# wenxiaoshuai/Points-Matching

Hardware: AMD Instinct MI355X
Metric: descriptor-pair distances/s (BF-L2 2-NN + ratio stage); RANSAC hypotheses/s in `ransac` (higher is better)
Workload: dtype f32

## Files before the change

### include/pm.h

```cpp
#ifndef PM_H_
#define PM_H_

#include <stddef.h>
#include <stdint.h>

#ifdef __cplusplus
extern "C" {
#endif

#define PM_VERSION_MAJOR 0
#define PM_VERSION_MINOR 1

typedef enum pm_status {
    PM_OK            =  0,
    PM_E_INVALID     = -1,
    PM_E_TOO_FEW     = -2,
    PM_E_NO_MODEL    = -3,
    PM_E_HIP         = -4,
    PM_E_NOMEM       = -5,
    PM_E_UNSUPPORTED = -6
} pm_status;

typedef struct pm_match {
    int32_t queryIdx;
    int32_t trainIdx;
    int32_t imgIdx;
    float   distance;
} pm_match;

typedef struct pm_ctx pm_ctx;

int  pm_ctx_create(int device, pm_ctx** out);
int  pm_ctx_destroy(pm_ctx* ctx);
int  pm_ctx_set_stream(pm_ctx* ctx, void* hip_stream);
int  pm_ctx_synchronize(pm_ctx* ctx);
int  pm_device_alloc(pm_ctx* ctx, size_t bytes, void** d_out);
int  pm_device_free(pm_ctx* ctx, void* d_ptr);
int  pm_device_upload(pm_ctx* ctx, void* d_dst, const void* src, size_t bytes);
int  pm_device_download(pm_ctx* ctx, void* dst, const void* d_src, size_t bytes);
int  pm_ctx_timing_enable(pm_ctx* ctx, int enable);
int  pm_ctx_timing_reset(pm_ctx* ctx);
int  pm_ctx_timing_get(pm_ctx* ctx, const char* kernel, double* mean_ms, int* launches);
int  pm_ctx_knn_diag_enable(pm_ctx* ctx, int enable);
int  pm_ctx_knn_stats(pm_ctx* ctx, int* rescans, int* nonfinite);
int  pm_ctx_knn_route(pm_ctx* ctx, int* route);
int  pm_ctx_filter_fusion_status(pm_ctx* ctx, int* gave_up);
enum {
    PM_OPT_RANSAC_PATH    = 1,
    PM_OPT_SCORE_OPERANDS = 2,
    PM_OPT_HAMMING_ROUTE  = 3,
    PM_OPT_KNN_F16_WAVES  = 4,
    PM_OPT_KNN_STAGING    = 6,
    PM_OPT_KNN_WG_PER_CU  = 7,
    PM_OPT_FILTER_FUSION  = 5,
    PM_OPT_KNN_XCD_TILE   = 8,
    PM_OPT_KNN_GENERAL_F16 = 9,
    PM_OPT_KNN_SEEDED     = 10,
    PM_OPT_KNN_U8_GROUP   = 11,
    PM_OPT_KNN_RING       = 12,
    PM_OPT_KNN_U8_REFINE  = 13,
    PM_OPT_KNN_RING_PROLOGUE = 14,
    PM_OPT_KNN_WIDE       = 15,
    PM_OPT_KNN_PREP_ROWS  = 16,
    PM_OPT_RANSAC_FORM    = 17,
    PM_OPT_RANSAC_WG_IDS  = 18,
    PM_OPT_HAMMING_REFINE = 19,
    PM_OPT_KNN_SUPERTILE  = 20,
    PM_OPT_FEAT_CAPACITY  = 21,
    PM_OPT_COUNT_         = 22
};
int  pm_ctx_set_option(pm_ctx* ctx, int option, int value);
int  pm_ctx_get_option(pm_ctx* ctx, int option, int* value);
const char* pm_last_error(void);
const char* pm_status_string(int status);
int  pm_version(void);

#define PM_MAX_K 16
#define PM_KNN_FORCE_EXACT  1
#define PM_KNN_FORCE_F32    2
#define PM_KNN_HINT_INTEGER 4
#define PM_KNN_HINT_U8      8
#define PM_KNN_HINT_UNIT_NORM 16
int pm_bf_knn_l2_f32(pm_ctx* ctx, const float* q, int nq, const float* t, int nt,
                     int dim, int k, int flags, pm_match* out);
int pm_bf_knn_l2_f32_dev(pm_ctx* ctx, const float* d_q, int nq, const float* d_t, int nt,
                         int dim, int k, int flags, pm_match* d_out);

int pm_bf_knn_l2_u8(pm_ctx* ctx, const uint8_t* q, int nq, const uint8_t* t, int nt, int dim, int k, pm_match* out);
int pm_bf_knn_l2_u8_dev(pm_ctx* ctx, const uint8_t* d_q, int nq, const uint8_t* d_t, int nt, int dim, int k, pm_match* d_out);
int pm_bf_knn_l2_u8_ratio_dev(pm_ctx* ctx, const uint8_t* d_q, int nq, const uint8_t* d_t, int nt, int dim, float ratio,
                              const float* d_kp1_xy, const float* d_kp2_xy, pm_match* d_knn, pm_match* d_good,
                              float* d_xy1, float* d_xy2, int32_t* d_n_good);

int pm_bf_knn_l2_ratio_dev(pm_ctx* ctx, const float* d_q, int nq, const float* d_t, int nt, int dim, int flags,
                           float ratio, const float* d_kp1_xy, const float* d_kp2_xy, pm_match* d_knn,
                           pm_match* d_good, float* d_xy1, float* d_xy2, int32_t* d_n_good);

typedef struct pm_flann_params {
    int32_t  trees;
    int32_t  checks;
    uint64_t seed;
} pm_flann_params;
typedef struct pm_flann_index pm_flann_index;
int pm_flann_build(pm_ctx* ctx, const float* train, int nt, int dim, const pm_flann_params* prm, pm_flann_index** out);
int pm_flann_destroy(pm_flann_index* ix);
int pm_flann_knn_l2_f32(pm_ctx* ctx, pm_flann_index* ix, const float* q, int nq, int k, pm_match* out);
int pm_flann_knn_l2_f32_dev(pm_ctx* ctx, pm_flann_index* ix, const float* d_q, int nq, int k, pm_match* d_out);
int pm_flann_export(const pm_flann_index* ix, int32_t* n_nodes, int32_t* roots, void* nodes, int32_t cap_nodes);

int pm_bf_knn_hamming_u8(pm_ctx* ctx, const uint8_t* q, int nq, const uint8_t* t, int nt,
                         int bytes, int k, pm_match* out);
int pm_bf_knn_hamming_u8_dev(pm_ctx* ctx, const uint8_t* d_q, int nq, const uint8_t* d_t, int nt,
                             int bytes, int k, pm_match* d_out);

int pm_pad_rows_u8(const uint8_t* src, int n, int bytes, uint8_t* dst, int dst_bytes);
int pm_pad_rows_u8_dev(pm_ctx* ctx, const uint8_t* d_src, int n, int bytes, uint8_t* d_dst, int dst_bytes);


int pm_filter_midpoint(const pm_match* m, int n, double* min_out, double* max_out,
                       pm_match* out, int* n_out);
int pm_filter_ratio(const pm_match* knn, int nq, int k, float ratio, pm_match* out, int* n_out);
int pm_filter_ratio_gather_dev(pm_ctx* ctx, const pm_match* d_knn, int nq, int k, float ratio,
// ... 311 lines not shown
```

### points_matching_amd/api.py

```python
import ctypes as C
import os

import numpy as np

_HERE = os.path.dirname(os.path.abspath(__file__))
LIB_PATH = os.environ.get("PM_LIB_PATH") or os.path.join(_HERE, "libpm_hip.so")

MATCH_DTYPE = np.dtype([("queryIdx", "<i4"), ("trainIdx", "<i4"), ("imgIdx", "<i4"),
                        ("distance", "<f4")])
PM_MAX_K = 16
PM_KNN_FORCE_EXACT = 1
PM_KNN_FORCE_F32 = 2
PM_KNN_HINT_INTEGER = 4
PM_KNN_HINT_U8 = 8
PM_KNN_HINT_UNIT_NORM = 16
PM_CROSS_RATIO_FWD = 1
PM_CROSS_RATIO_REV = 2
PM_GUIDE_F_SAMPSON = 0
PM_GUIDE_F_SYM = 1
PM_GUIDE_H = 2
PM_ERR_SAMPSON = 0
PM_ERR_SYM_EPIPOLAR = 1
PM_ERR_REPROJ = 2
PM_AFFINE_FULL = 0
# ... 54 lines not shown
    _fields_ = [("hyp_begin", C.c_int64), ("hyp_end", C.c_int64), ("seed", C.c_uint64),
                ("thresh_px", C.c_float), ("error_kind", C.c_int32)]


class PointsView(C.Structure):
    _fields_ = [("xy1", C.c_void_p), ("xy2", C.c_void_p), ("counts", C.c_void_p), ("parts", C.c_int32),
                ("cap", C.c_int32), ("pitch_xy", C.c_int64), ("pitch_cnt", C.c_int32), ("reserved", C.c_int32)]


class Camera(C.Structure):
    _fields_ = [("fx", C.c_double), ("fy", C.c_double), ("cx", C.c_double), ("cy", C.c_double)]


def _camera(K):
    if isinstance(K, Camera):
        return K
    k = np.asarray(K, np.float64)
    if k.shape == (3, 3):
        return Camera(k[0, 0], k[1, 1], k[0, 2], k[1, 2])
    return Camera(*[float(v) for v in k.reshape(4)])


class PnpView(C.Structure):
    _fields_ = [("xyz", C.c_void_p), ("uv", C.c_void_p), ("count", C.c_void_p), ("cap", C.c_int32), ("reserved", C.c_int32)]


class HRefineInfo(C.Structure):
    _fields_ = [("cost_in", C.c_double), ("cost_out", C.c_double), ("n_used", C.c_int32), ("iters", C.c_int32),
                ("status", C.c_int32), ("reserved", C.c_int32)]


H_REFINE_INFO_DTYPE = np.dtype([("cost_in", "<f8"), ("cost_out", "<f8"), ("n_used", "<i4"), ("iters", "<i4"),
                                ("status", "<i4"), ("reserved", "<i4")])

RANSAC_RECORD_DTYPE = np.dtype([("key", "<u8"), ("F", "<f8", (9,))])
PM_MAX_PARTS = 64
PM_OPT_RANSAC_PATH, PM_OPT_SCORE_OPERANDS, PM_OPT_HAMMING_ROUTE, PM_OPT_KNN_F16_WAVES, PM_OPT_FILTER_FUSION = 1, 2, 3, 4, 5
PM_OPT_KNN_STAGING = 6
PM_OPT_KNN_WG_PER_CU = 7
PM_OPT_KNN_XCD_TILE = 8
PM_OPT_KNN_GENERAL_F16 = 9
PM_OPT_KNN_SEEDED = 10
PM_OPT_KNN_U8_GROUP = 11
PM_OPT_KNN_RING = 12
PM_OPT_KNN_U8_REFINE = 13
PM_OPT_KNN_RING_PROLOGUE = 14
PM_OPT_KNN_WIDE = 15
PM_OPT_KNN_PREP_ROWS = 16
PM_OPT_RANSAC_FORM = 17
PM_OPT_RANSAC_WG_IDS = 18
PM_OPT_HAMMING_REFINE = 19
PM_OPT_KNN_SUPERTILE = 20
PM_OPT_FEAT_CAPACITY = 21


_lib = None


def lib():
    global _lib
    if _lib is None:
        if not os.path.exists(LIB_PATH):
            raise PmError(PM_E_UNSUPPORTED,
                          "%s is missing: run `python -m points_matching_amd.build`" % LIB_PATH)
        try:
            import torch
        except ImportError:
            pass
        _lib = C.CDLL(LIB_PATH)
        _lib.pm_last_error.restype = C.c_char_p
        _lib.pm_status_string.restype = C.c_char_p
        _lib.pm_format_match_list.restype = C.c_long
    return _lib


def _check(rc):
    if rc != PM_OK:
        raise PmError(rc, (lib().pm_last_error() or b"").decode() or
                      lib().pm_status_string(rc).decode())


def _p(a):
    return a.ctypes.data_as(C.c_void_p) if a is not None else None


def _pair(xy1, xy2):
    xy1 = np.ascontiguousarray(xy1, np.float32).reshape(-1, 2)
    xy2 = np.ascontiguousarray(xy2, np.float32).reshape(-1, 2)
    if xy2.shape[0] != xy1.shape[0]:
        raise ValueError("xy1 and xy2 must have the same length")
    return xy1, xy2, xy1.shape[0]


def _outcome(rc):
    if rc not in (PM_OK, PM_E_NO_MODEL, PM_E_TOO_FEW):
        _check(rc)
    return rc


def ransac_key(inliers, hyp):
    return (int(inliers) << 32) | (0xFFFFFFFF - int(hyp))


def ransac_key_hyp(key):
    return 0xFFFFFFFF - (int(key) & 0xFFFFFFFF)

# ... 1016 lines not shown
```

### points_matching_amd/csrc/ransac_fused_kernels.hpp

```cpp
#pragma once
#include <type_traits>

#include "ransac_core.hpp"
#include "ransac_internal.hpp"

namespace pm_ransac {
namespace {

constexpr int RF_THREADS = 256;
constexpr int RF_TEAMS = 2;
constexpr int RF_WG = RF_THREADS * RF_TEAMS;
constexpr int RF_PTS_PER_SLOT = 2 * RF_THREADS;
constexpr int RF_PPT2 = 5;
constexpr int RF_PPT2_BIG = 10;
static_assert(RF_PPT2_BIG <= 10, "score_tile is instantiated for 1..10 slots");

struct RfSlot {
    unsigned long long key;
    double F[9];
    unsigned long long pad[6];
};
static_assert(sizeof(RfSlot) == 128, "slot stride");

struct RfOut {
    int shard;
    unsigned long long* key;
    double* F;
    uint8_t* mask;
    int mask_len;
    int* n_inliers;
    FinalOut* fo;
    union {
        pm_ransac_record* rec;
        const double* cand;
    };
};

__device__ __forceinline__ int view_count1(const pm_points_view& v)
{
    int c = v.cap;
    if (v.counts) { const int raw = *v.counts; c = raw < 0 ? 0 : (raw > v.cap ? v.cap : raw); }
    return c;
}
__device__ __forceinline__ void view_offsets(const pm_points_view& v, int* __restrict__ offs, int tid)
{
    if (tid < 64) {
        int c = 0;
        if (tid < v.parts) {
            c = v.cap;
            if (v.counts) {
                const int raw = v.counts[static_cast<size_t>(tid) * v.pitch_cnt];
                c = raw < 0 ? 0 : (raw > v.cap ? v.cap : raw);
            }
        }
        int incl = c;
#pragma unroll
        for (int o = 1; o < 64; o <<= 1) {
            const int up = __shfl_up(incl, o, 64);
            if (tid >= o) incl += up;
        }
        if (tid < v.parts) offs[tid] = incl - c;
        if (tid == v.parts - 1) offs[v.parts] = incl;
    }
}

__device__ __forceinline__ void view_point(const pm_points_view& v, const int* __restrict__ offs, int i, float2& a, float2& b)
{
    size_t e = 2 * static_cast<size_t>(i);
    if (v.parts > 1) {
        int p = 0;
        while (p + 1 < v.parts && i >= offs[p + 1]) ++p;
        e = static_cast<size_t>(p) * static_cast<size_t>(v.pitch_xy) + 2 * static_cast<size_t>(i - offs[p]);
    }
    a = *reinterpret_cast<const float2*>(v.xy1 + e);
    b = *reinterpret_cast<const float2*>(v.xy2 + e);
}

template <typename DIAG>
__device__ __forceinline__ bool hyp_model_view(const pm_points_view& v, const int* __restrict__ offs, int n, uint64_t seed,
                                               uint64_t h, double (&F)[9])
{
    int idx[8];
    DIAG::solve(5);
    sample8(seed, h, n, idx);
    DIAG::solve(6);
    double x1[8], y1[8], x2[8], y2[8];
#pragma unroll
    for (int i = 0; i < 8; ++i) {
        float2 a, b;
// ... 95 lines not shown
                                           const f32x2 (&YP)[PPT2], float thr2, bool first, int lane, int wave, int team)
{
    if (team >= hcount) return;
    f32x4v m0 = *reinterpret_cast<const f32x4v*>(&mdl[team][0]);
    f32x4v m1 = *reinterpret_cast<const f32x4v*>(&mdl[team][4]);
    f32x2 m2 = *reinterpret_cast<const f32x2*>(&mdl[team][8]);
    for (int s = team; s < hcount; s += RF_TEAMS) {
        const f32x4v c0 = m0, c1 = m1;
        const f32x2 c2 = m2;
        const int sn = s + RF_TEAMS < hcount ? s + RF_TEAMS : s;
        m0 = *reinterpret_cast<const f32x4v*>(&mdl[sn][0]);
        m1 = *reinterpret_cast<const f32x4v*>(&mdl[sn][4]);
        m2 = *reinterpret_cast<const f32x2*>(&mdl[sn][8]);
        const ModelS ms = model_to_sgprs(c0, c1, c2);
        unsigned long long va[KM], vb[KM];
        const float fs[9] = {c0[0], c0[1], c0[2], c0[3], c1[0], c1[1], c1[2], c1[3], c2[0]};
#pragma unroll
        for (int k = 0; k < KM; ++k) {
            bool ia, ib;
            if constexpr (DIAG::scalar_fma) {
                ia = inlier32<KIND>(fs, X[k][0], Y[k][0], XP[k][0], YP[k][0], thr2);
                ib = inlier32<KIND>(fs, X[k][1], Y[k][1], XP[k][1], YP[k][1], thr2);
            } else {
                inlier_pk_model<KIND>(ms, X[k], Y[k], XP[k], YP[k], thr2, ia, ib);
            }
            va[k] = __ballot(ia);
            vb[k] = __ballot(ib);
        }
        int c = 0;
#pragma unroll
        for (int k = 0; k < KM; ++k) c += __popcll(va[k]) + __popcll(vb[k]);
        if (lane == 0) {
            if (first) cnt[wave][s] = c;
            else __hip_atomic_fetch_add(&cnt[wave][s], c, __ATOMIC_RELAXED, __HIP_MEMORY_SCOPE_WORKGROUP);
        }
    }
}

template <int NWAVES>
__device__ __forceinline__ unsigned long long wg_max_u64(unsigned long long key, unsigned long long* __restrict__ wk, int tid)
{
    key = pm::wave_max_u64(key);
    __syncthreads();
    if ((tid & 63) == 0) wk[tid >> 6] = key;
    __syncthreads();
    unsigned long long k = wk[0];
#pragma unroll
    for (int w = 1; w < NWAVES; ++w) k = wk[w] > k ? wk[w] : k;
    return k;
}

template <int KIND, int PPT2, typename DIAG>
__global__ __launch_bounds__(RF_WG) void ransac_fused(pm_points_view v, uint64_t seed, int64_t hyp_begin, int nh, int hb,
                                                           float thr2, RfSlot* __restrict__ slots, int* __restrict__ ticket,
                                                           RfOut out)
{
    __shared__ __attribute__((aligned(16))) float s_mdl[RF_HB_MAX][12];
    __shared__ double s_m64[RF_HB_MAX][9];
    __shared__ int s_cnt[RF_THREADS / 64][RF_HB_MAX];
    __shared__ int s_offs[PM_MAX_PARTS + 1];
    __shared__ unsigned long long s_wk[RF_WG / 64];
    __shared__ double s_F64[9];
    __shared__ int s_role;
    __shared__ int s_wc[RF_THREADS / 64];

    const int tid = threadIdx.x, lane = tid & 63, wave = tid >> 6;
    const int team = tid / RF_THREADS, ttid = tid % RF_THREADS, twave = wave % (RF_THREADS / 64);
    DIAG::phase(0);
    int n;
    if (v.parts == 1) {
        n = view_count1(v);
    } else {
        view_offsets(v, s_offs, tid);
        __syncthreads();
        n = s_offs[v.parts];
    }
    DIAG::phase(1);

    constexpr int RF_TILE = RF_PTS_PER_SLOT * PPT2;
    const int ntiles = n > RF_TILE ? (n + RF_TILE - 1) / RF_TILE : 1;
    f32x2 X[PPT2], Y[PPT2], XP[PPT2], YP[PPT2];
    const float nanv = __builtin_nanf("");
    auto load_tile = [&](int t) -> int {
        const int base = t * RF_TILE;
        int kmax = (n - base + RF_PTS_PER_SLOT - 1) / RF_PTS_PER_SLOT;
        kmax = kmax < 0 ? 0 : (kmax > PPT2 ? PPT2 : kmax);
#pragma unroll
        for (int k = 0; k < PPT2; ++k) {
            X[k] = f32x2{nanv, nanv}; Y[k] = X[k]; XP[k] = X[k]; YP[k] = X[k];
            if (k < kmax) {
                const int i0 = base + 2 * (k * RF_THREADS + ttid);
                float2 a0 = {nanv, nanv}, b0 = a0, a1 = a0, b1 = a0;
                if (v.parts == 1) {
                    const int j0 = i0 < n ? i0 : n - 1, j1 = i0 + 1 < n ? i0 + 1 : n - 1;
                    a0 = *reinterpret_cast<const float2*>(v.xy1 + 2 * static_cast<size_t>(j0));
                    a1 = *reinterpret_cast<const float2*>(v.xy1 + 2 * static_cast<size_t>(j1));
                    b0 = *reinterpret_cast<const float2*>(v.xy2 + 2 * static_cast<size_t>(j0));
                    b1 = *reinterpret_cast<const float2*>(v.xy2 + 2 * static_cast<size_t>(j1));
                    if (i0 >= n) { a0 = float2{nanv, nanv}; b0 = a0; }
                    if (i0 + 1 >= n) { a1 = float2{nanv, nanv}; b1 = a1; }
                } else {
                    if (i0 < n) view_point(v, s_offs, i0, a0, b0);
                    if (i0 + 1 < n) view_point(v, s_offs, i0 + 1, a1, b1);
                }
                X[k] = f32x2{a0.x, a1.x}; Y[k] = f32x2{a0.y, a1.y};
                XP[k] = f32x2{b0.x, b1.x}; YP[k] = f32x2{b0.y, b1.y};
            }
        }
        return kmax;
    };
    DIAG::phase(2);

    const int h0 = static_cast<int>(blockIdx.x) * hb;
    const int hcount = nh - h0 < hb ? nh - h0 : hb;
    if (tid < hcount) {
        double F[9];
        bool ok = false;
#pragma unroll
        for (int i = 0; i < 9; ++i) F[i] = 0.0;
        if (n >= 8) ok = hyp_model_view<DIAG>(v, s_offs, n, seed, static_cast<uint64_t>(hyp_begin + h0 + tid), F);
#pragma unroll
        for (int i = 0; i < 9; ++i) { s_mdl[tid][i] = static_cast<float>(F[i]); s_m64[tid][i] = F[i]; }
        s_mdl[tid][9] = ok ? 1.f : 0.f;
        s_mdl[tid][10] = 0.f; s_mdl[tid][11] = 0.f;
    }
    DIAG::phase(3);
    int kmax = load_tile(0);
    __syncthreads();
    DIAG::phase(4);

    for (int t = 0; t < ntiles; ++t) {
        if (t > 0) kmax = load_tile(t);
        switch (kmax) {
#define PM_CASE(KM_) case KM_: score_tile<KIND, PPT2, (KM_ <= PPT2 ? KM_ : PPT2), DIAG>(s_mdl, s_cnt, hcount, X, Y, XP, YP, thr2, t == 0, lane, twave, team); break;
            PM_CASE(1) PM_CASE(2) PM_CASE(3) PM_CASE(4) PM_CASE(5) PM_CASE(6) PM_CASE(7) PM_CASE(8) PM_CASE(9) PM_CASE(10)
#undef PM_CASE
            default:
                if (team == 0) for (int s = lane; s < hcount; s += 64) s_cnt[twave][s] = t == 0 ? 0 : s_cnt[twave][s];
                break;
        }
    }
    DIAG::phase(5);
    __syncthreads();

    unsigned long long key = 0ull;
    if (tid < hcount && s_mdl[tid][9] != 0.f) {
        int c = 0;
#pragma unroll
        for (int w = 0; w < RF_THREADS / 64; ++w) c += s_cnt[w][tid];
        key = (static_cast<unsigned long long>(static_cast<uint32_t>(c)) << 32) |
              static_cast<unsigned long long>(0xFFFFFFFFu - static_cast<uint32_t>(hyp_begin + h0 + tid));
    }
    const unsigned long long kbest = wg_max_u64<RF_WG / 64>(key, s_wk, tid);
    if (wave == 0) {
        const int sb = kbest ? static_cast<int>(static_cast<int64_t>(0xFFFFFFFFu - static_cast<uint32_t>(kbest)) - hyp_begin) - h0 : 0;
        RfSlot* sl = slots + blockIdx.x;
        if (lane < 9) __hip_atomic_store(&sl->F[lane], kbest ? s_m64[sb][lane] : 0.0, __ATOMIC_RELAXED, __HIP_MEMORY_SCOPE_AGENT);
        if (lane == 9) __hip_atomic_store(&sl->key, kbest, __ATOMIC_RELAXED, __HIP_MEMORY_SCOPE_AGENT);
        asm volatile("s_waitcnt vmcnt(0)" ::: "memory");
        if (lane == 0) {
            const int tk = __hip_atomic_fetch_add(ticket, 1, __ATOMIC_RELAXED, __HIP_MEMORY_SCOPE_AGENT);
            s_role = tk == static_cast<int>(gridDim.x) - 1 ? 1 : 0;
        }
    }
    __syncthreads();
    DIAG::phase(6);
    if (s_role == 0) { DIAG::phase(9); return; }

    if (tid == 0) __hip_atomic_store(ticket, 0, __ATOMIC_RELAXED, __HIP_MEMORY_SCOPE_AGENT);
    unsigned long long kb = 0ull;
    double fb[9];
#pragma unroll
    for (int i = 0; i < 9; ++i) fb[i] = 0.0;
    for (int j = tid; j < static_cast<int>(gridDim.x); j += RF_WG) {
        const unsigned long long kj = __hip_atomic_load(&slots[j].key, __ATOMIC_RELAXED, __HIP_MEMORY_SCOPE_AGENT);
        double fj[9];
#pragma unroll
        for (int i = 0; i < 9; ++i) fj[i] = __hip_atomic_load(&slots[j].F[i], __ATOMIC_RELAXED, __HIP_MEMORY_SCOPE_AGENT);
        if (kj > kb) {
            kb = kj;
#pragma unroll
            for (int i = 0; i < 9; ++i) fb[i] = fj[i];
        }
    }
    const unsigned long long kwin = wg_max_u64<RF_WG / 64>(kb, s_wk, tid);
    const bool ok = kwin != 0ull && n >= 8;
    if (tid < 9) s_F64[tid] = 0.0;
    __syncthreads();
    if (ok && kb == kwin) {
#pragma unroll
        for (int i = 0; i < 9; ++i) s_F64[i] = fb[i];
    }
    __syncthreads();
    DIAG::phase(7);
    if (out.shard) {
        if (tid < 9) out.rec->F[tid] = s_F64[tid];
        if (tid == 9) out.rec->key = ok ? kwin : 0ull;
        return;
    }
    if (tid < 9) {
        if (out.F) out.F[tid] = s_F64[tid];
        if (out.fo) { out.fo->F[tid] = s_F64[tid]; out.fo->F32[tid] = static_cast<float>(s_F64[tid]); }
    }
    if (tid == 9) {
        *out.key = ok ? kwin : 0ull;
        if (out.fo) out.fo->valid = ok ? 1 : 0;
    }
    float fw[9];
#pragma unroll
    for (int i = 0; i < 9; ++i) fw[i] = static_cast<float>(s_F64[i]);
    int mine = 0;
    if (team == 0) {
        for (int t = 0; t < ntiles; ++t) {
            if (ntiles > 1) kmax = load_tile(t);
#pragma unroll
            for (int k = 0; k < PPT2; ++k) {
                if (k < kmax) {
                    bool ia, ib;
                    inlier32_x2_flags<KIND>(fw, X[k], Y[k], XP[k], YP[k], thr2, ia, ib);
                    ia = ia && ok; ib = ib && ok;
                    const int i0 = t * RF_TILE + 2 * (k * RF_THREADS + ttid);
                    if (i0 < out.mask_len) out.mask[i0] = ia ? 1 : 0;
                    if (i0 + 1 < out.mask_len) out.mask[i0 + 1] = ib ? 1 : 0;
                    mine += __popcll(__ballot(ia)) + __popcll(__ballot(ib));
                }
            }
        }
        if (lane == 0) s_wc[twave] = mine;
    }
    const int covered = n > 0 ? (n + RF_PTS_PER_SLOT - 1) / RF_PTS_PER_SLOT * RF_PTS_PER_SLOT : 0;
    for (int i = covered + tid; i < out.mask_len; i += RF_WG) out.mask[i] = 0;
    __syncthreads();
    if (tid == 0) {
        int tot = 0;
#pragma unroll
        for (int w = 0; w < RF_THREADS / 64; ++w) tot += s_wc[w];
        if (out.n_inliers) *out.n_inliers = tot;
        if (out.fo) out.fo->n_inliers = tot;
    }
    DIAG::phase(8);
    DIAG::phase(9);
}

constexpr int RL_WAVES = 12;
constexpr int RL_THREADS = RL_WAVES * 64;
constexpr int RL_SLOT_PTS = 128;
constexpr int RL_MAX_SLOTS = 64;

struct GeomF {
    static constexpr bool OWN = false;
    static constexpr int PLANES = 4, MW = 12, FLAG = 9, WORDS = 9, MAX_SLOTS = RL_MAX_SLOTS;
};
template <typename M, typename = void>
struct GeomOf {
    using type = GeomF;
};
template <typename M>
struct GeomOf<M, std::void_t<typename M::Geom>> {
    using type = typename M::Geom;
};

template <typename MODEL, int NH>
__device__ __forceinline__ void score_lds(const float (*s_mdl)[12], int* s_cnt, const f32x2* pp, int kslots, int s0, float thr2, int lane)
{
    ModelS ms[NH];
    int c[NH];
#pragma unroll
    for (int h = 0; h < NH; ++h) {
        const float* m = s_mdl[s0 + h * RL_WAVES];
        ms[h] = model_to_sgprs(*reinterpret_cast<const f32x4v*>(m), *reinterpret_cast<const f32x4v*>(m + 4),
                               *reinterpret_cast<const f32x2*>(m + 8));
        c[h] = 0;
    }
    for (int slot = 0; slot < kslots; ++slot) {
        const f32x2 x = pp[0], y = pp[64], xp = pp[128], yp = pp[192];
        pp += 256;
#pragma unroll
        for (int h = 0; h < NH; ++h) {
            bool ia, ib;
            MODEL::inlier_pk(ms[h], x, y, xp, yp, thr2, ia, ib);
            c[h] += __popcll(__ballot(ia)) + __popcll(__ballot(ib));
        }
    }
    if (lane == 0) {
// ... 10 lines not shown
        typename MODEL::Regs ms[NH];
        int c[NH];
#pragma unroll
        for (int h = 0; h < NH; ++h) {
            ms[h] = MODEL::regs(s_mdl[ss[h]]);
            c[h] = 0;
        }
        for (int slot = 0; slot < kslots; ++slot) {
            f32x2 op[G::PLANES];
#pragma unroll
            for (int q = 0; q < G::PLANES; ++q) op[q] = pp[64 * q];
            pp += 64 * G::PLANES;
#pragma unroll
            for (int h = 0; h < NH; ++h) {
                bool ia, ib;
                MODEL::inlier_pk(ms[h], op, thr2, ia, ib);
                c[h] += __popcll(__ballot(ia)) + __popcll(__ballot(ib));
            }
        }
        if (lane == 0) {
#pragma unroll
            for (int h = 0; h < NH; ++h) s_cnt[ss[h]] += c[h];
        }
    } else {
        ModelS ms[NH];
        int c[NH];
#pragma unroll
        for (int h = 0; h < NH; ++h) {
            const float* m = s_mdl[ss[h]];
            ms[h] = model_to_sgprs(*reinterpret_cast<const f32x4v*>(m), *reinterpret_cast<const f32x4v*>(m + 4),
                                   *reinterpret_cast<const f32x2*>(m + 8));
            c[h] = 0;
        }
        for (int slot = 0; slot < kslots; ++slot) {
            const f32x2 x = pp[0], y = pp[64], xp = pp[128], yp = pp[192];
            pp += 256;
#pragma unroll
            for (int h = 0; h < NH; ++h) {
                bool ia, ib;
                MODEL::inlier_pk(ms[h], x, y, xp, yp, thr2, ia, ib);
                c[h] += __popcll(__ballot(ia)) + __popcll(__ballot(ib));
            }
        }
        if (lane == 0) {
#pragma unroll
            for (int h = 0; h < NH; ++h) s_cnt[ss[h]] += c[h];
        }
    }
}

template <typename MODEL, typename DIAG>
__global__ __launch_bounds__(RL_THREADS) void ransac_fused_lds(pm_points_view v, uint64_t seed, int64_t hyp_begin, int nh, int hb,
                                                               float thr2, int tile_slots, RfSlot* __restrict__ slots,
                                                               int* __restrict__ ticket, RfOut out)
{
    using G = typename GeomOf<MODEL>::type;
    extern __shared__ __attribute__((aligned(16))) f32x2 s_pts[];
    __shared__ __attribute__((aligned(16))) float s_mdl[RF_HB_MAX][G::MW];
    __shared__ double s_m64[RF_HB_MAX][G::WORDS];
    __shared__ int s_cnt[RF_HB_MAX];
    __shared__ int s_offs[PM_MAX_PARTS + 1];
    __shared__ unsigned long long s_wk[RL_WAVES];
    __shared__ double s_F64[G::WORDS];
    __shared__ int s_role;
    __shared__ int s_wc[RL_WAVES];

    const int tid = threadIdx.x, lane = tid & 63, wave = tid >> 6;
    DIAG::phase(0);
    int n;
    if (v.parts == 1) {
        n = view_count1(v);
    } else {
        view_offsets(v, s_offs, tid);
        __syncthreads();
        n = s_offs[v.parts];
    }
    DIAG::phase(1);
    const int tile_pts = tile_slots * RL_SLOT_PTS;
    const int ntiles = n > tile_pts ? (n + tile_pts - 1) / tile_pts : 1;
    const float nanv = __builtin_nanf("");
    auto load_pair = [&](int base, int slot, int l) {
        const int i0 = base + 2 * (64 * slot + l);
        if constexpr (G::OWN) {
            MODEL::load_pair(v, n, i0, s_pts + static_cast<size_t>(slot) * G::PLANES * 64 + l);
        } else {
            float2 a0 = {nanv, nanv}, b0 = a0, a1 = a0, b1 = a0;
            if (v.parts == 1) {
                if (n > 0) {
                    const int j0 = i0 < n ? i0 : n - 1, j1 = i0 + 1 < n ? i0 + 1 : n - 1;
                    a0 = *reinterpret_cast<const float2*>(v.xy1 + 2 * static_cast<size_t>(j0));
                    a1 = *reinterpret_cast<const float2*>(v.xy1 + 2 * static_cast<size_t>(j1));
                    b0 = *reinterpret_cast<const float2*>(v.xy2 + 2 * static_cast<size_t>(j0));
                    b1 = *reinterpret_cast<const float2*>(v.xy2 + 2 * static_cast<size_t>(j1));
                }
                if (i0 >= n) { a0 = float2{nanv, nanv}; b0 = a0; }
                if (i0 + 1 >= n) { a1 = float2{nanv, nanv}; b1 = a1; }
            } else {
                if (i0 < n) view_point(v, s_offs, i0, a0, b0);
                if (i0 + 1 < n) view_point(v, s_offs, i0 + 1, a1, b1);
            }
            f32x2* d = s_pts + (static_cast<size_t>(slot) * 4) * 64 + l;
            d[0] = f32x2{a0.x, a1.x}; d[64] = f32x2{a0.y, a1.y}; d[128] = f32x2{b0.x, b1.x}; d[192] = f32x2{b0.y, b1.y};
        }
    };
    auto tile_kslots = [&](int t) {
        int k = (n - t * tile_pts + RL_SLOT_PTS - 1) / RL_SLOT_PTS;
        return k < 0 ? 0 : (k > tile_slots ? tile_slots : k);
// ... 43 lines not shown

    for (int t = 0; t < ntiles; ++t) {
        const int kslots = tile_kslots(t);
        if (t > 0) {
            __syncthreads();
            for (int slot = wave; slot < kslots; slot += RL_WAVES) load_pair(t * tile_pts, slot, lane);
            __syncthreads();
        }
        if constexpr (MODEL::CANDIDATES) {
            const int sk = wave + RL_WAVES * lane;
            unsigned long long live = __ballot(sk < hcount && s_mdl[sk < hcount ? sk : 0][G::FLAG] != 0.f);
            while (live) {
                int ss[4];
                int k = 0;
#pragma unroll
                for (int h = 0; h < 4; ++h) {
                    ss[h] = wave;
                    if (live) {
                        ss[h] = wave + RL_WAVES * static_cast<int>(__builtin_ctzll(live));
                        live &= live - 1;
                        k = h + 1;
                    }
                }
                if (k == 4) score_lds_ids<MODEL, 4, G>(s_mdl, s_cnt, s_pts + lane, kslots, ss, thr2, lane);
                else if (k == 3) score_lds_ids<MODEL, 3, G>(s_mdl, s_cnt, s_pts + lane, kslots, ss, thr2, lane);
                else if (k == 2) score_lds_ids<MODEL, 2, G>(s_mdl, s_cnt, s_pts + lane, kslots, ss, thr2, lane);
                else score_lds_ids<MODEL, 1, G>(s_mdl, s_cnt, s_pts + lane, kslots, ss, thr2, lane);
            }
        } else {
            for (int s = wave; s < hcount; s += 4 * RL_WAVES) {
                const int left = (hcount - s + RL_WAVES - 1) / RL_WAVES;
                if (left >= 4) score_lds<MODEL, 4>(s_mdl, s_cnt, s_pts + lane, kslots, s, thr2, lane);
                else if (left == 3) score_lds<MODEL, 3>(s_mdl, s_cnt, s_pts + lane, kslots, s, thr2, lane);
                else if (left == 2) score_lds<MODEL, 2>(s_mdl, s_cnt, s_pts + lane, kslots, s, thr2, lane);
                else score_lds<MODEL, 1>(s_mdl, s_cnt, s_pts + lane, kslots, s, thr2, lane);
            }
        }
    }
    DIAG::phase(5);
    __syncthreads();

    unsigned long long key = 0ull;
    if (tid < hcount && s_mdl[tid][G::FLAG] != 0.f)
        key = (static_cast<unsigned long long>(static_cast<uint32_t>(s_cnt[tid])) << 32) |
              static_cast<unsigned long long>(0xFFFFFFFFu - static_cast<uint32_t>(hyp_begin + h0 + tid));
    const unsigned long long kbest = wg_max_u64<RL_WAVES>(key, s_wk, tid);
    if (wave == 0) {
        const int sb = kbest ? static_cast<int>(static_cast<int64_t>(0xFFFFFFFFu - static_cast<uint32_t>(kbest)) - hyp_begin) - h0 : 0;
        double* sf = reinterpret_cast<double*>(slots) + static_cast<size_t>(lane) * gridDim.x + blockIdx.x;
        if (lane < G::WORDS) __hip_atomic_store(sf, kbest ? s_m64[sb][lane] : 0.0, __ATOMIC_RELAXED, __HIP_MEMORY_SCOPE_AGENT);
        if (lane == G::WORDS) __hip_atomic_store(reinterpret_cast<unsigned long long*>(sf), kbest, __ATOMIC_RELAXED, __HIP_MEMORY_SCOPE_AGENT);
        asm volatile("s_waitcnt vmcnt(0)" ::: "memory");
        if (lane == 0) {
            const int tk = __hip_atomic_fetch_add(ticket, 1, __ATOMIC_RELAXED, __HIP_MEMORY_SCOPE_AGENT);
            s_role = tk == static_cast<int>(gridDim.x) - 1 ? 1 : 0;
        }
    }
    __syncthreads();
    DIAG::phase(6);
    if (s_role == 0) { DIAG::phase(9); return; }

    if (tid == 0) __hip_atomic_store(ticket, 0, __ATOMIC_RELAXED, __HIP_MEMORY_SCOPE_AGENT);
    unsigned long long kb = 0ull;
    double fb[G::WORDS];
#pragma unroll
    for (int i = 0; i < G::WORDS; ++i) fb[i] = 0.0;
    for (int j = tid; j < static_cast<int>(gridDim.x); j += RL_THREADS) {
        const double* sf = reinterpret_cast<const double*>(slots) + j;
        const unsigned long long kj = __hip_atomic_load(reinterpret_cast<const unsigned long long*>(sf + G::WORDS * static_cast<size_t>(gridDim.x)),
                                                        __ATOMIC_RELAXED, __HIP_MEMORY_SCOPE_AGENT);
        double fj[G::WORDS];
#pragma unroll
        for (int i = 0; i < G::WORDS; ++i) fj[i] = __hip_atomic_load(sf + i * static_cast<size_t>(gridDim.x), __ATOMIC_RELAXED, __HIP_MEMORY_SCOPE_AGENT);
        if (kj > kb) {
            kb = kj;
#pragma unroll
            for (int i = 0; i < G::WORDS; ++i) fb[i] = fj[i];
        }
    }
    const unsigned long long kwin = wg_max_u64<RL_WAVES>(kb, s_wk, tid);
    const bool ok = kwin != 0ull && n >= MODEL::MIN_PTS;
    if (tid < G::WORDS) s_F64[tid] = 0.0;
    __syncthreads();
    if (ok && kb == kwin) {
#pragma unroll
        for (int i = 0; i < G::WORDS; ++i) s_F64[i] = fb[i];
    }
    __syncthreads();
    DIAG::phase(7);
    if (MODEL::SHARD_OUT && out.shard) {
        if (tid < 9) out.rec->F[tid] = s_F64[tid];
        if (tid == 9) out.rec->key = ok ? kwin : 0ull;
        return;
    }
    if (tid < G::WORDS) {
        if (out.F && (MODEL::OUT_WORDS == G::WORDS || tid < MODEL::OUT_WORDS)) out.F[tid] = s_F64[tid];
        if (MODEL::SHARD_OUT && out.fo) { out.fo->F[tid] = s_F64[tid]; out.fo->F32[tid] = static_cast<float>(s_F64[tid]); }
    }
    if (tid == G::WORDS) {
        *out.key = ok ? kwin : 0ull;
        if (MODEL::SHARD_OUT && out.fo) out.fo->valid = ok ? 1 : 0;
    }
    float fw[G::OWN ? G::MW : 9];
    if constexpr (G::OWN) {
        MODEL::mask_model(out.cand, ok, kwin, hyp_begin, fw);
    } else {
#pragma unroll
        for (int i = 0; i < 9; ++i) fw[i] = static_cast<float>(s_F64[i]);
    }
    int mine = 0;
    for (int t = 0; t < ntiles; ++t) {
        const int kslots = tile_kslots(t);
        if (ntiles > 1) {
            __syncthreads();
            for (int slot = wave; slot < kslots; slot += RL_WAVES) load_pair(t * tile_pts, slot, lane);
            __syncthreads();
        }
        for (int slot = wave; slot < kslots; slot += RL_WAVES) {
            const f32x2* pp = s_pts + static_cast<size_t>(slot) * (64 * G::PLANES) + lane;
            bool ia, ib;
            if constexpr (G::OWN) {
                f32x2 op[G::PLANES];
#pragma unroll
                for (int q = 0; q < G::PLANES; ++q) op[q] = pp[64 * q];
                MODEL::inlier_x2(fw, op, thr2, ia, ib);
            } else {
                MODEL::inlier_x2(fw, pp[0], pp[64], pp[128], pp[192], thr2, ia, ib);
            }
            ia = ia && ok; ib = ib && ok;
            const int i0 = t * tile_pts + 2 * (64 * slot + lane);
            if (i0 < out.mask_len) out.mask[i0] = ia ? 1 : 0;
            if (i0 + 1 < out.mask_len) out.mask[i0 + 1] = ib ? 1 : 0;
            mine += __popcll(__ballot(ia)) + __popcll(__ballot(ib));
        }
    }
    if (lane == 0) s_wc[wave] = mine;
    const int covered = n > 0 ? (n + RL_SLOT_PTS - 1) / RL_SLOT_PTS * RL_SLOT_PTS : 0;
    for (int i = covered + tid; i < out.mask_len; i += RL_THREADS) out.mask[i] = 0;
    __syncthreads();
    if (tid == 0) {
        int tot = 0;
#pragma unroll
        for (int w = 0; w < RL_WAVES; ++w) tot += s_wc[w];
        if (out.n_inliers) *out.n_inliers = tot;
        if (MODEL::SHARD_OUT && out.fo) out.fo->n_inliers = tot;
    }
    DIAG::phase(8);
    DIAG::phase(9);
}

int sync_words(pm_ctx* ctx, int** out)
{
    if (!ctx->sync_words) {
        PM_HIP_CHECK(hipMalloc(reinterpret_cast<void**>(&ctx->sync_words), 256));
        PM_HIP_CHECK(hipMemsetAsync(ctx->sync_words, 0, 256, ctx->stream));
    }
    *out = ctx->sync_words;
    return PM_OK;
}

template <typename MODEL, typename DIAG>
int fused_lds_launch(pm_ctx* ctx, const pm_points_view& v, const pm_ransac_params* p, int nwg, int hb, RfSlot* slots,
                     int* ticket, const RfOut& out)
{
    using G = typename GeomOf<MODEL>::type;
    const long long cap_total = static_cast<long long>(v.parts) * v.cap;
    const long long need = (cap_total + RL_SLOT_PTS - 1) / RL_SLOT_PTS;
    const int tile_slots = static_cast<int>(need < 1 ? 1 : (need > G::MAX_SLOTS ? G::MAX_SLOTS : need));
    const size_t lds = static_cast<size_t>(tile_slots) * G::PLANES * 64 * sizeof(f32x2);
    static bool attr_done_dev[PM_MAX_DEVICES] = {};
    if (!attr_done_dev[ctx->device]) {
        PM_HIP_CHECK(hipFuncSetAttribute(reinterpret_cast<const void*>(&ransac_fused_lds<MODEL, DIAG>),
                                         hipFuncAttributeMaxDynamicSharedMemorySize,
                                         G::MAX_SLOTS * G::PLANES * 64 * static_cast<int>(sizeof(f32x2))));
        attr_done_dev[ctx->device] = true;
    }
    const float thr2 = p->thresh_px * p->thresh_px;
    hipLaunchKernelGGL((ransac_fused_lds<MODEL, DIAG>), dim3(nwg), dim3(RL_THREADS), lds, ctx->stream, v, p->seed, p->hyp_begin,
                       static_cast<int>(p->hyp_end - p->hyp_begin), hb, thr2, tile_slots, slots, ticket, out);
    PM_HIP_CHECK(hipGetLastError());
    return PM_OK;
}

template <typename MODEL>
int fused_lds_enqueue(pm_ctx* ctx, const pm_points_view& v, const pm_ransac_params* p, int sync_word, const char* timer,
                      unsigned long long* d_key, double* d_model, uint8_t* d_mask, int mask_len, int* d_ninl,
                      const double* d_cand = nullptr)
{
    const long long nh = p->hyp_end - p->hyp_begin;
    const int hb = fused_hb(ctx, nh);
    const int nwg = static_cast<int>((nh + hb - 1) / hb);
    RfSlot* slots = static_cast<RfSlot*>(pm::arena_take(ctx, sizeof(RfSlot) * static_cast<size_t>(nwg)));
    PM_REQUIRE(slots, PM_E_NOMEM, "scratch arena too small");
    int* sync = nullptr;
    int rc = sync_words(ctx, &sync);
    if (rc != PM_OK) return rc;
    RfOut out{};
    out.key = d_key; out.F = d_model; out.mask = d_mask; out.mask_len = mask_len; out.n_inliers = d_ninl;
    out.cand = d_cand;
    pm::ScopedKernelTime t(ctx, timer);
    return fused_lds_launch<MODEL, NoDiag>(ctx, v, p, nwg, hb, slots, sync + sync_word, out);
}

template <typename DIAG>
int fused_launch_t(pm_ctx* ctx, const pm_points_view& v, const pm_ransac_params* p, int shard, pm_ransac_record* d_rec,
                 unsigned long long* d_key, double* d_F, uint8_t* d_mask, int mask_len, int* d_ninl, FinalOut** fo_out)
{
    const long long nh = p->hyp_end - p->hyp_begin;
    const long long cap_total = static_cast<long long>(v.parts) * v.cap;
    PM_REQUIRE(nh >= 1, PM_E_INVALID, "fused_launch: empty hypothesis range");
    PM_REQUIRE(nh <= 0x7FFFFFFFLL, PM_E_INVALID, "a single launch takes at most 2^31 - 1 hypothesis ids: split the range");
    const int hb = fused_hb(ctx, nh);
    const int nwg = static_cast<int>((nh + hb - 1) / hb);
    RfSlot* slots = static_cast<RfSlot*>(pm::arena_take(ctx, sizeof(RfSlot) * static_cast<size_t>(nwg)));
    FinalOut* fo = static_cast<FinalOut*>(pm::arena_take(ctx, sizeof(FinalOut)));
    PM_REQUIRE(slots && fo, PM_E_NOMEM, "scratch arena too small");
    int* sync = nullptr;
    int rc = sync_words(ctx, &sync);
    if (rc != PM_OK) return rc;
    RfOut out{};
    out.shard = shard;
    out.key = d_key; out.F = d_F; out.mask = d_mask; out.mask_len = mask_len; out.n_inliers = d_ninl;
    out.fo = fo_out ? fo : nullptr;
    out.rec = d_rec;
    if (fo_out) *fo_out = fo;
    const float thr2 = p->thresh_px * p->thresh_px;
    pm::ScopedKernelTime t(ctx, "ransac_fused");
    if (ctx->opts[PM_OPT_RANSAC_FORM] != 1) {
        if (p->error_kind == PM_ERR_SAMPSON) return fused_lds_launch<FModel<PM_ERR_SAMPSON>, DIAG>(ctx, v, p, nwg, hb, slots, sync, out);
        return fused_lds_launch<FModel<PM_ERR_SYM_EPIPOLAR>, DIAG>(ctx, v, p, nwg, hb, slots, sync, out);
    }
#define PM_RF(KIND_, PPT2_)                                                                                              \
    hipLaunchKernelGGL((ransac_fused<KIND_, PPT2_, DIAG>), dim3(nwg), dim3(RF_WG), 0, ctx->stream, v, p->seed, p->hyp_begin, \
                       static_cast<int>(nh), hb, thr2, slots, sync, out)
    const int depth = cap_total <= 2 * RF_PTS_PER_SLOT ? 2 : (cap_total <= RF_PPT2 * RF_PTS_PER_SLOT ? RF_PPT2 : RF_PPT2_BIG);
#define PM_RF_K(KIND_)                                                                   \
    do {                                                                                 \
        if (depth == 2) PM_RF(KIND_, 2);                                                 \
        else if (depth == RF_PPT2) PM_RF(KIND_, RF_PPT2);                                \
        else PM_RF(KIND_, RF_PPT2_BIG);                                                  \
    } while (0)
    if (p->error_kind == PM_ERR_SAMPSON) PM_RF_K(PM_ERR_SAMPSON);
    else PM_RF_K(PM_ERR_SYM_EPIPOLAR);
#undef PM_RF_K
#undef PM_RF
    PM_HIP_CHECK(hipGetLastError());
    return PM_OK;
}

}
}
```

Baseline: 2272 billion.

## Add sharded two-level completion ticket and wider RANSAC mask stores

Adds an optional two-level ticket: workgroups first increment one of eight counters, each on its own padded line, and only the last arrival per shard bumps a top counter, which is meant to cut contention on a single global atomic. It also writes inlier-mask pairs as 16-bit stores when the mask is aligned and zero-fills the mask tail with 16-byte stores. The sharded ticket only turns on by default above 2^30 workgroups, so unless the option is forced it stays off and the default path keeps the single atomic; the mask-store changes always apply. The sync-word buffer grows to hold the ticket blocks.

New measurement: 2270 billion. About the same (-0.1%).

```diff
diff --git a/include/pm.h b/include/pm.h
--- a/include/pm.h
+++ b/include/pm.h
@@ -67,7 +67,8 @@
     PM_OPT_HAMMING_REFINE = 19,
     PM_OPT_KNN_SUPERTILE  = 20,
     PM_OPT_FEAT_CAPACITY  = 21,
-    PM_OPT_COUNT_         = 22
+    PM_OPT_RANSAC_TICKET  = 22,
+    PM_OPT_COUNT_         = 23
 };
 int  pm_ctx_set_option(pm_ctx* ctx, int option, int value);
 int  pm_ctx_get_option(pm_ctx* ctx, int option, int* value);
diff --git a/points_matching_amd/api.py b/points_matching_amd/api.py
--- a/points_matching_amd/api.py
+++ b/points_matching_amd/api.py
@@ -130,6 +130,7 @@
 PM_OPT_HAMMING_REFINE = 19
 PM_OPT_KNN_SUPERTILE = 20
 PM_OPT_FEAT_CAPACITY = 21
+PM_OPT_RANSAC_TICKET = 22
 
 
 _lib = None
diff --git a/points_matching_amd/csrc/ransac_fused_kernels.hpp b/points_matching_amd/csrc/ransac_fused_kernels.hpp
--- a/points_matching_amd/csrc/ransac_fused_kernels.hpp
+++ b/points_matching_amd/csrc/ransac_fused_kernels.hpp
@@ -35,6 +35,73 @@
         const double* cand;
     };
 };
+
+constexpr int RF_TICKET_SHARDS = 8;
+constexpr int RF_TICKET_LINE = 32;
+constexpr int RF_TICKET_BLOCK = (RF_TICKET_SHARDS + 1) * RF_TICKET_LINE;
+constexpr int RF_TICKET_BLOCKS = 5;
+constexpr int RF_SYNC_LEGACY = 64;
+constexpr int RF_SYNC_INTS = RF_SYNC_LEGACY + RF_TICKET_BLOCKS * RF_TICKET_BLOCK;
+constexpr int RF_TICKET_SHARD_MIN = 1 << 30;
+
+__host__ __device__ constexpr int ticket_pop(int nwg, int s) { return s < nwg ? (nwg - s + RF_TICKET_SHARDS - 1) / RF_TICKET_SHARDS : 0; }
+__host__ __device__ constexpr int ticket_top_pop(int nwg) { return nwg < RF_TICKET_SHARDS ? nwg : RF_TICKET_SHARDS; }
+constexpr int ticket_pop_sum(int nwg)
+{
+    int t = 0;
+    for (int s = 0; s < RF_TICKET_SHARDS; ++s) t += ticket_pop(nwg, s);
+    return t;
+}
+static_assert(ticket_pop_sum(1) == 1 && ticket_pop_sum(7) == 7 && ticket_pop_sum(8) == 8 && ticket_pop_sum(9) == 9, "shard populations");
+static_assert(ticket_pop_sum(63) == 63 && ticket_pop_sum(64) == 64 && ticket_pop_sum(65) == 65, "shard populations");
+static_assert(ticket_pop_sum(250) == 250 && ticket_pop_sum(782) == 782, "shard populations");
+constexpr int ticket_block(int sync_word) { return sync_word == 0 ? 0 : sync_word / 4 - 1; }
+static_assert(ticket_block(8) == 1 && ticket_block(12) == 2 && ticket_block(16) == 3 && ticket_block(20) == RF_TICKET_BLOCKS - 1, "ticket blocks");
+
+struct RfTicket {
+    int* word;
+    int two;
+};
+
+__device__ __forceinline__ bool ticket_draw(const RfTicket& tk, int nwg, int b)
+{
+    if (!tk.two) return __hip_atomic_fetch_add(tk.word, 1, __ATOMIC_RELAXED, __HIP_MEMORY_SCOPE_AGENT) == nwg - 1;
+    const int s = b & (RF_TICKET_SHARDS - 1);
+    int* sh = tk.word + s * RF_TICKET_LINE;
+    if (__hip_atomic_fetch_add(sh, 1, __ATOMIC_RELAXED, __HIP_MEMORY_SCOPE_AGENT) != ticket_pop(nwg, s) - 1) return false;
+    __hip_atomic_store(sh, 0, __ATOMIC_RELAXED, __HIP_MEMORY_SCOPE_AGENT);
+    int* top = tk.word + RF_TICKET_SHARDS * RF_TICKET_LINE;
+    return __hip_atomic_fetch_add(top, 1, __ATOMIC_RELAXED, __HIP_MEMORY_SCOPE_AGENT) == ticket_top_pop(nwg) - 1;
+}
+__device__ __forceinline__ void ticket_reset(const RfTicket& tk)
+{
+    __hip_atomic_store(tk.two ? tk.word + RF_TICKET_SHARDS * RF_TICKET_LINE : tk.word, 0, __ATOMIC_RELAXED, __HIP_MEMORY_SCOPE_AGENT);
+}
+
+__device__ __forceinline__ void mask_store_pair(uint8_t* __restrict__ mask, int mask_len, bool pair_ok, int i0, bool ia, bool ib)
+{
+    if (pair_ok && i0 + 1 < mask_len) {
+        *reinterpret_cast<uint16_t*>(mask + i0) = static_cast<uint16_t>((ia ? 1u : 0u) | (ib ? 0x100u : 0u));
+    } else {
+        if (i0 < mask_len) mask[i0] = ia ? 1 : 0;
+        if (i0 + 1 < mask_len) mask[i0 + 1] = ib ? 1 : 0;
+    }
+}
+template <int THREADS>
+__device__ __forceinline__ void mask_zero_fill(uint8_t* __restrict__ mask, int from, int mask_len, int tid)
+{
+    const int len = mask_len - from;
+    if (len <= 0) return;
+    uint8_t* p = mask + from;
+    int head = static_cast<int>((16u - static_cast<unsigned>(reinterpret_cast<uintptr_t>(p) & 15u)) & 15u);
+    head = head < len ? head : len;
+    const int n16 = (len - head) >> 4;
+    const int tail0 = head + (n16 << 4);
+    if (tid < head) p[tid] = 0;
+    uint4* q = reinterpret_cast<uint4*>(p + head);
+    for (int j = tid; j < n16; j += THREADS) q[j] = uint4{0u, 0u, 0u, 0u};
+    if (tid < len - tail0) p[tail0 + tid] = 0;
+}
 
 __device__ __forceinline__ int view_count1(const pm_points_view& v)
 {
@@ -236,7 +303,7 @@
 
 template <int KIND, int PPT2, typename DIAG>
 __global__ __launch_bounds__(RF_WG) void ransac_fused(pm_points_view v, uint64_t seed, int64_t hyp_begin, int nh, int hb,
-                                                           float thr2, RfSlot* __restrict__ slots, int* __restrict__ ticket,
+                                                           float thr2, RfSlot* __restrict__ slots, RfTicket ticket,
                                                            RfOut out)
 {
     __shared__ __attribute__((aligned(16))) float s_mdl[RF_HB_MAX][12];
@@ -343,15 +410,14 @@
         if (lane == 9) __hip_atomic_store(&sl->key, kbest, __ATOMIC_RELAXED, __HIP_MEMORY_SCOPE_AGENT);
         asm volatile("s_waitcnt vmcnt(0)" ::: "memory");
         if (lane == 0) {
-            const int tk = __hip_atomic_fetch_add(ticket, 1, __ATOMIC_RELAXED, __HIP_MEMORY_SCOPE_AGENT);
-            s_role = tk == static_cast<int>(gridDim.x) - 1 ? 1 : 0;
+            s_role = ticket_draw(ticket, static_cast<int>(gridDim.x), static_cast<int>(blockIdx.x)) ? 1 : 0;
         }
     }
     __syncthreads();
     DIAG::phase(6);
     if (s_role == 0) { DIAG::phase(9); return; }
 
-    if (tid == 0) __hip_atomic_store(ticket, 0, __ATOMIC_RELAXED, __HIP_MEMORY_SCOPE_AGENT);
+    if (tid == 0) ticket_reset(ticket);
     unsigned long long kb = 0ull;
     double fb[9];
 #pragma unroll
@@ -394,6 +460,7 @@
 #pragma unroll
     for (int i = 0; i < 9; ++i) fw[i] = static_cast<float>(s_F64[i]);
     int mine = 0;
+    const bool pair_ok = (reinterpret_cast<uintptr_t>(out.mask) & 1u) == 0;
     if (team == 0) {
         for (int t = 0; t < ntiles; ++t) {
             if (ntiles > 1) kmax = load_tile(t);
@@ -404,8 +471,7 @@
                     inlier32_x2_flags<KIND>(fw, X[k], Y[k], XP[k], YP[k], thr2, ia, ib);
                     ia = ia && ok; ib = ib && ok;
                     const int i0 = t * RF_TILE + 2 * (k * RF_THREADS + ttid);
-                    if (i0 < out.mask_len) out.mask[i0] = ia ? 1 : 0;
-                    if (i0 + 1 < out.mask_len) out.mask[i0 + 1] = ib ? 1 : 0;
+                    mask_store_pair(out.mask, out.mask_len, pair_ok, i0, ia, ib);
                     mine += __popcll(__ballot(ia)) + __popcll(__ballot(ib));
                 }
             }
@@ -413,7 +479,7 @@
         if (lane == 0) s_wc[twave] = mine;
     }
     const int covered = n > 0 ? (n + RF_PTS_PER_SLOT - 1) / RF_PTS_PER_SLOT * RF_PTS_PER_SLOT : 0;
-    for (int i = covered + tid; i < out.mask_len; i += RF_WG) out.mask[i] = 0;
+    mask_zero_fill<RF_WG>(out.mask, covered, out.mask_len, tid);
     __syncthreads();
     if (tid == 0) {
         int tot = 0;
@@ -530,7 +596,7 @@
 template <typename MODEL, typename DIAG>
 __global__ __launch_bounds__(RL_THREADS) void ransac_fused_lds(pm_points_view v, uint64_t seed, int64_t hyp_begin, int nh, int hb,
                                                                float thr2, int tile_slots, RfSlot* __restrict__ slots,
-                                                               int* __restrict__ ticket, RfOut out)
+                                                               RfTicket ticket, RfOut out)
 {
     using G = typename GeomOf<MODEL>::type;
     extern __shared__ __attribute__((aligned(16))) f32x2 s_pts[];
@@ -680,15 +746,14 @@
         if (lane == G::WORDS) __hip_atomic_store(reinterpret_cast<unsigned long long*>(sf), kbest, __ATOMIC_RELAXED, __HIP_MEMORY_SCOPE_AGENT);
         asm volatile("s_waitcnt vmcnt(0)" ::: "memory");
         if (lane == 0) {
-            const int tk = __hip_atomic_fetch_add(ticket, 1, __ATOMIC_RELAXED, __HIP_MEMORY_SCOPE_AGENT);
-            s_role = tk == static_cast<int>(gridDim.x) - 1 ? 1 : 0;
+            s_role = ticket_draw(ticket, static_cast<int>(gridDim.x), static_cast<int>(blockIdx.x)) ? 1 : 0;
         }
     }
     __syncthreads();
     DIAG::phase(6);
     if (s_role == 0) { DIAG::phase(9); return; }
 
-    if (tid == 0) __hip_atomic_store(ticket, 0, __ATOMIC_RELAXED, __HIP_MEMORY_SCOPE_AGENT);
+    if (tid == 0) ticket_reset(ticket);
     unsigned long long kb = 0ull;
     double fb[G::WORDS];
 #pragma unroll
@@ -737,6 +802,7 @@
         for (int i = 0; i < 9; ++i) fw[i] = static_cast<float>(s_F64[i]);
     }
     int mine = 0;
+    const bool pair_ok = (reinterpret_cast<uintptr_t>(out.mask) & 1u) == 0;
     for (int t = 0; t < ntiles; ++t) {
         const int kslots = tile_kslots(t);
         if (ntiles > 1) {
@@ -757,14 +823,13 @@
             }
             ia = ia && ok; ib = ib && ok;
             const int i0 = t * tile_pts + 2 * (64 * slot + lane);
-            if (i0 < out.mask_len) out.mask[i0] = ia ? 1 : 0;
-            if (i0 + 1 < out.mask_len) out.mask[i0 + 1] = ib ? 1 : 0;
+            mask_store_pair(out.mask, out.mask_len, pair_ok, i0, ia, ib);
             mine += __popcll(__ballot(ia)) + __popcll(__ballot(ib));
         }
     }
     if (lane == 0) s_wc[wave] = mine;
     const int covered = n > 0 ? (n + RL_SLOT_PTS - 1) / RL_SLOT_PTS * RL_SLOT_PTS : 0;
-    for (int i = covered + tid; i < out.mask_len; i += RL_THREADS) out.mask[i] = 0;
+    mask_zero_fill<RL_THREADS>(out.mask, covered, out.mask_len, tid);
     __syncthreads();
     if (tid == 0) {
         int tot = 0;
@@ -780,16 +845,23 @@
 int sync_words(pm_ctx* ctx, int** out)
 {
     if (!ctx->sync_words) {
-        PM_HIP_CHECK(hipMalloc(reinterpret_cast<void**>(&ctx->sync_words), 256));
-        PM_HIP_CHECK(hipMemsetAsync(ctx->sync_words, 0, 256, ctx->stream));
+        PM_HIP_CHECK(hipMalloc(reinterpret_cast<void**>(&ctx->sync_words), sizeof(int) * RF_SYNC_INTS));
+        PM_HIP_CHECK(hipMemsetAsync(ctx->sync_words, 0, sizeof(int) * RF_SYNC_INTS, ctx->stream));
     }
     *out = ctx->sync_words;
     return PM_OK;
 }
 
+inline RfTicket ticket_of(const pm_ctx* ctx, int* sync, int sync_word, int nwg)
+{
+    const int opt = ctx->opts[PM_OPT_RANSAC_TICKET];
+    const bool two = opt == 2 || (opt != 1 && nwg >= RF_TICKET_SHARD_MIN);
+    return two ? RfTicket{sync + RF_SYNC_LEGACY + ticket_block(sync_word) * RF_TICKET_BLOCK, 1} : RfTicket{sync + sync_word, 0};
+}
+
 template <typename MODEL, typename DIAG>
 int fused_lds_launch(pm_ctx* ctx, const pm_points_view& v, const pm_ransac_params* p, int nwg, int hb, RfSlot* slots,
-                     int* ticket, const RfOut& out)
+                     const RfTicket& ticket, const RfOut& out)
 {
     using G = typename GeomOf<MODEL>::type;
     const long long cap_total = static_cast<long long>(v.parts) * v.cap;
@@ -827,7 +899,7 @@
     out.key = d_key; out.F = d_model; out.mask = d_mask; out.mask_len = mask_len; out.n_inliers = d_ninl;
     out.cand = d_cand;
     pm::ScopedKernelTime t(ctx, timer);
-    return fused_lds_launch<MODEL, NoDiag>(ctx, v, p, nwg, hb, slots, sync + sync_word, out);
+    return fused_lds_launch<MODEL, NoDiag>(ctx, v, p, nwg, hb, slots, ticket_of(ctx, sync, sync_word, nwg), out);
 }
 
 template <typename DIAG>
@@ -853,14 +925,15 @@
     out.rec = d_rec;
     if (fo_out) *fo_out = fo;
     const float thr2 = p->thresh_px * p->thresh_px;
+    const RfTicket ticket = ticket_of(ctx, sync, 0, nwg);
     pm::ScopedKernelTime t(ctx, "ransac_fused");
     if (ctx->opts[PM_OPT_RANSAC_FORM] != 1) {
-        if (p->error_kind == PM_ERR_SAMPSON) return fused_lds_launch<FModel<PM_ERR_SAMPSON>, DIAG>(ctx, v, p, nwg, hb, slots, sync, out);
-        return fused_lds_launch<FModel<PM_ERR_SYM_EPIPOLAR>, DIAG>(ctx, v, p, nwg, hb, slots, sync, out);
+        if (p->error_kind == PM_ERR_SAMPSON) return fused_lds_launch<FModel<PM_ERR_SAMPSON>, DIAG>(ctx, v, p, nwg, hb, slots, ticket, out);
+        return fused_lds_launch<FModel<PM_ERR_SYM_EPIPOLAR>, DIAG>(ctx, v, p, nwg, hb, slots, ticket, out);
     }
 #define PM_RF(KIND_, PPT2_)                                                                                              \
     hipLaunchKernelGGL((ransac_fused<KIND_, PPT2_, DIAG>), dim3(nwg), dim3(RF_WG), 0, ctx->stream, v, p->seed, p->hyp_begin, \
-                       static_cast<int>(nh), hb, thr2, slots, sync, out)
+                       static_cast<int>(nh), hb, thr2, slots, ticket, out)
     const int depth = cap_total <= 2 * RF_PTS_PER_SLOT ? 2 : (cap_total <= RF_PPT2 * RF_PTS_PER_SLOT ? RF_PPT2 : RF_PPT2_BIG);
 #define PM_RF_K(KIND_)                                                                   \
     do {                                                                                 \
```
